# nelilepo/timetabling-ga-mpi-openmp

Hardware: AMD Instinct MI355X
Metric: fitness evals/sec (hcv+scv), pop 64K, 400-event instance; 1/2/4/8 GPUs (higher is better)
Workload: dtype i32; 1 GPU; med instance E=400 R=10 F=5 S=200 (seeded synthetic, medium01-size), population 65536 per GPU, one tt_eval (hcv+scv+feasible+penalty) per step; pop_per_gpu=65536, global_pop=65536, kernel=eval_tile5_w8, parallelism=dp1 (independent population shards)

## Files before the change

### timetabling-ga-mpi-openmp_amd/csrc/tt_common.h

```cpp
#pragma once
#include <hip/hip_runtime.h>
#include <stdint.h>

namespace ttga {

constexpr int kSlots = 45;
constexpr int kSlotsPerDay = 9;
constexpr int kMaxRooms = 64;
constexpr int kMaxSlotEvents = 256;

constexpr uint64_t kLastSlotMask = (1ull << 8) | (1ull << 17) | (1ull << 26) | (1ull << 35) | (1ull << 44);
constexpr uint64_t kTripleMask = 0x7Full | (0x7Full << 9) | (0x7Full << 18) | (0x7Full << 27) | (0x7Full << 36);

struct DevProblem {
    int E, R, S, EW;
    const int32_t* sn;
    const int32_t* stu_off;
    const int32_t* stu_ev;
    const int32_t* ev_off;
    const int32_t* ev_stu;
    const uint64_t* poss;
    const uint32_t* corr;
    int EW64;
    const uint64_t* cupT;
    const uint64_t* corr64;
    const int32_t* stc_off;
    const int32_t* stc_ev;
    const uint32_t* sid;
    const int4* srun;
    const int32_t* srun_part;
    int32_t* status;
};
constexpr int kSrunPart4 = 0, kSrunPart8 = 5, kSrunPart16 = 14, kSrunPartLen = 32;
__host__ __device__ constexpr int srun_part_base(int nw) { return nw == 4 ? kSrunPart4 : nw == 8 ? kSrunPart8 : kSrunPart16; }

__device__ __forceinline__ double pm_next(int64_t& s) {
    const int64_t IA = 16807, IM = 2147483647, IQ = 127773, IR = 2836;
    const double AM = 1.0 / 2147483647.0;
    if ((uint64_t)s <= 0x7FFFFFFFull) {
        const uint32_t u = (uint32_t)s;
        const uint32_t k32 = u / 127773u;
        int32_t t = 16807 * (int32_t)(u - k32 * 127773u) - 2836 * (int32_t)k32;
        if (t < 0) t += 2147483647;
        s = t;
        return __dmul_rn(AM, (double)t);
    }
    int64_t k = s / IQ;
    s = IA * (s - k * IQ) - IR * k;
    if (s < 0) s += IM;
    return __dmul_rn(AM, (double)s);
}

constexpr uint32_t kPmM = 2147483647u;
__device__ __forceinline__ uint32_t pm_mulmod(uint32_t a, uint32_t b) {
    const uint64_t p = (uint64_t)a * b;
    const uint32_t r = (uint32_t)(p & kPmM) + (uint32_t)(p >> 31);
    return r >= kPmM ? r - kPmM : r;
}
__device__ __forceinline__ uint32_t pm_pow(int n) {
    uint32_t r = 1, b = 16807u;
    for (; n; n >>= 1) {
        if (n & 1) r = pm_mulmod(r, b);
        b = pm_mulmod(b, b);
    }
    return r;
}

__device__ __forceinline__ int pm_pick(int64_t& s, int n) { return (int)__dmul_rn(pm_next(s), (double)n); }

__device__ __forceinline__ int mask_scv(uint64_t m) {
    int sc = __popcll(m & (m >> 1) & (m >> 2) & kTripleMask);
#pragma unroll
    for (int d = 0; d < 5; ++d) sc += (__popc((uint32_t)(m >> (9 * d)) & 0x1FFu) == 1);
    return sc;
}

__device__ __forceinline__ int wave_sum(int v) {
    v += __builtin_amdgcn_update_dpp(0, v, 0x111, 0xf, 0xf, true);
    v += __builtin_amdgcn_update_dpp(0, v, 0x112, 0xf, 0xf, true);
    v += __builtin_amdgcn_update_dpp(0, v, 0x114, 0xf, 0xf, true);
    v += __builtin_amdgcn_update_dpp(0, v, 0x118, 0xf, 0xf, true);
    v += __builtin_amdgcn_update_dpp(0, v, 0x142, 0xa, 0xf, false);
    v += __builtin_amdgcn_update_dpp(0, v, 0x143, 0xc, 0xf, false);
    return __builtin_amdgcn_readlane(v, 63);
}

__device__ __forceinline__ uint64_t ballot(bool p) { return __builtin_amdgcn_ballot_w64(p); }
__device__ __forceinline__ bool wave_any(bool p) { return __builtin_amdgcn_ballot_w64(p) != 0ull; }

__device__ __forceinline__ int wave_id() { return __builtin_amdgcn_readfirstlane((int)(threadIdx.x >> 6)); }

}
```

### timetabling-ga-mpi-openmp_amd/csrc/tt_derive.hip

```cpp
#include <hip/hip_runtime.h>

#include "tt_internal.h"

namespace ttga {
namespace {

typedef int v4i __attribute__((ext_vector_type(4)));
typedef int v16i __attribute__((ext_vector_type(16)));

__device__ __forceinline__ v4i bits_to_bytes(uint32_t h16) {
    v4i v;
#pragma unroll
    for (int d = 0; d < 4; d++) v[d] = (int)((__builtin_amdgcn_ubfe(h16, 4 * d, 4) * 0x00204081u) & 0x01010101u);
    return v;
}

struct DeriveOut {
    uint32_t* corr;
    uint32_t* corr64;
    uint32_t* cupT;
    int32_t* sn;
    uint64_t* poss;
};

// ... 44 lines not shown
    uint32_t myrow = 0u;
    uint32_t colbits = 0u;
#pragma unroll
    for (int g = 0; g < 16; g++) {
        const bool nz = acc[g] > 0;
        const uint64_t bal = ballot(nz);
        if (lane == acc_row(g, 0)) myrow = (uint32_t)bal;
        if (lane == acc_row(g, 1)) myrow = (uint32_t)(bal >> 32);
        if (nz) colbits |= 1u << acc_row(g, h);
    }
    const uint32_t col = colbits | (uint32_t)__shfl_xor((int)colbits, 32);
    if (lane < 32) {
        put_row_word(o, E, EW, EW64, i0 + lane, j0, myrow);
        if (!(diag_block && qi == qj)) put_row_word(o, E, EW, EW64, j0 + lane, i0, col);
    }
    if (diag_block && qi == qj) {
        const int c = r;
        if (h == ((c >> 2) & 1)) {
            const int reg = (c & 3) + 4 * (c >> 3);
            int v = 0;
#pragma unroll
            for (int g = 0; g < 16; g++) if (g == reg) v = acc[g];
            const int e = i0 + c;
            if (e < E) {
                o.sn[e] = v;
                uint64_t pm = 0ull;
                for (int rr = 0; rr < R; rr++) {
                    if (room_size[rr] < v) continue;
                    bool ok = true;
                    for (int f = 0; f < FW; f++) ok &= (efw[(size_t)e * FW + f] & ~rfw[(size_t)rr * FW + f]) == 0ull;
                    if (ok) pm |= 1ull << rr;
                }
                o.poss[e] = pm;
            }
        }
    }
}

}

int derive_on_device(const tt_problem* p, const uint32_t* atb, const int32_t* room_size, const uint64_t* efw,
                     const uint64_t* rfw, int FW) {
    const int E = p->E, S = p->S, R = p->R;
    const DeriveLayout DL = derive_layout(E, S);
    const int nb = DL.Ep / 64;
    const size_t at_bytes = ((size_t)DL.Ep * DL.SW * 4 + 255) & ~(size_t)255;
    const size_t rs_bytes = 256 * ((sizeof(int32_t) * R + 255) / 256);
    const size_t ef_bytes = ((sizeof(uint64_t) * E * FW) + 255) & ~(size_t)255;
    const size_t rf_bytes = ((sizeof(uint64_t) * R * FW) + 255) & ~(size_t)255;
    const size_t total = at_bytes + rs_bytes + ef_bytes + rf_bytes + 256;
    uint8_t* tmp = nullptr;
    hipStream_t st = nullptr;
    TT_HIP(hipStreamCreateWithFlags(&st, hipStreamNonBlocking));
    hipError_t he = hipMalloc(&tmp, total);
    if (he == hipErrorOutOfMemory) {
        (void)hipGetLastError();
        (void)hipStreamDestroy(st);
        set_error("tt_problem_create: the " + std::to_string(total >> 20) +
                  " MiB derivation image (E x S attendance bits) does not fit in device memory");
        return TT_ERR_LIMIT;
    }
    if (he != hipSuccess) { (void)hipStreamDestroy(st); return check_hip(he, "derive: hipMalloc"); }
    uint32_t* dAt = (uint32_t*)tmp;
    int32_t* drs = (int32_t*)(tmp + at_bytes);
    uint64_t* def = (uint64_t*)((uint8_t*)drs + rs_bytes);
    uint64_t* drf = (uint64_t*)((uint8_t*)def + ef_bytes);
    const DevProblem& d = p->dev;
    DeriveOut o{const_cast<uint32_t*>(d.corr), (uint32_t*)const_cast<uint64_t*>(d.corr64),
                (uint32_t*)const_cast<uint64_t*>(d.cupT), const_cast<int32_t*>(d.sn), const_cast<uint64_t*>(d.poss)};
    if (DL.SW > 0) he = hipMemcpyAsync(dAt, atb, (size_t)DL.Ep * DL.SW * 4, hipMemcpyHostToDevice, st);
    if (he == hipSuccess) he = hipMemcpyAsync(drs, room_size, sizeof(int32_t) * R, hipMemcpyHostToDevice, st);
    if (he == hipSuccess && FW > 0) he = hipMemcpyAsync(def, efw, sizeof(uint64_t) * E * FW, hipMemcpyHostToDevice, st);
    if (he == hipSuccess && FW > 0) he = hipMemcpyAsync(drf, rfw, sizeof(uint64_t) * R * FW, hipMemcpyHostToDevice, st);
    if (he == hipSuccess)
        hipLaunchKernelGGL(derive_corr_kernel, dim3(nb * (nb + 1) / 2), dim3(256), 0, st, dAt, E, DL.Sp, nb, drs, R, def,
                           drf, FW, o);
    if (he == hipSuccess) he = hipGetLastError();
    if (he == hipSuccess) he = hipStreamSynchronize(st);
    (void)hipFree(tmp);
    (void)hipStreamDestroy(st);
    return check_hip(he, "derive_on_device");
}

}
```

### timetabling-ga-mpi-openmp_amd/csrc/tt_eval.hip

```cpp
#include <algorithm>
#include <type_traits>
#include <utility>
#include <vector>

#include "tt_internal.h"

namespace ttga {

typedef __attribute__((address_space(4))) const uint32_t ConstU32;
typedef __attribute__((address_space(4))) const int32_t ConstI32;
typedef __attribute__((address_space(3))) unsigned long long LdsU64;


__device__ __forceinline__ int bcnt_acc(uint32_t x, int acc) {
    int r;
    asm("v_bcnt_u32_b32 %0, %1, %2" : "=v"(r) : "v"(x), "v"(acc));
    return r;
}
__device__ __forceinline__ int popc_acc(uint64_t x, int acc) {
    int r, t;
    asm("v_bcnt_u32_b32 %0, %1, %2" : "=v"(t) : "v"((uint32_t)x), "v"(acc));
    asm("v_bcnt_u32_b32 %0, %1, %2" : "=v"(r) : "v"((uint32_t)(x >> 32)), "v"(t));
    return r;
}
// ... 154 lines not shown
        }
    }
    if constexpr (K == 2) {
        if (cnt & 1) {
            uint32_t r[N / 2];
            sload_rec<N / 2>(q + steps * ST, r);
            sc += students_scv<N, 1, GAP>(my, r);
        }
    }
    return sc;
}
__device__ __noinline__ int run_scv_any(const uint8_t* my, const ConstU32* p, int cnt, int n, bool gap) {
    int sc = 0;
    for (int i = 0; i < cnt; ++i) {
        uint64_t m = 0;
        for (int j = 0; j < n / 2; ++j) {
            const uint32_t d = p[i * (n / 2) + j];
            m |= 1ull << (my[d & 0xFFFFu] & 63);
            m |= 1ull << (my[d >> 16] & 63);
        }
        sc += gap ? mask_scv_gap(m) : mask_scv(m);
    }
    return sc;
}
template <int KMAX, bool GAP = false>
__device__ __forceinline__ int lane_scv_runs(const uint8_t* my, const DevProblem& pb, int r0, int r1) {
    const ConstI32* runs = (const ConstI32*)pb.srun;
    int sc = 0;
    for (int k = r0; k < r1; ++k) {
        const int n = runs[4 * k], off = runs[4 * k + 1], cnt = runs[4 * k + 2];
        const uint32_t* p = pb.sid + off;
        switch (n) {
#define TT_RUN(N) case N: sc += run_scv<N, KMAX, GAP>(my, p, cnt); break;
            TT_RUN(2) TT_RUN(4) TT_RUN(6) TT_RUN(8) TT_RUN(10) TT_RUN(12) TT_RUN(14) TT_RUN(16)
            TT_RUN(18) TT_RUN(20) TT_RUN(22) TT_RUN(24) TT_RUN(26) TT_RUN(28) TT_RUN(30) TT_RUN(32)
#undef TT_RUN
            default: sc += run_scv_any(my, (const ConstU32*)p, cnt, n, GAP); break;
        }
    }
    return sc;
}

#ifndef TT_EVAL_ABLATE
#define TT_EVAL_ABLATE 0
#endif
__host__ __device__ inline int t5_cnt_bytes(int R) {
    return kSlots * ((R + 1) / 2) * 4;
}

struct Tile5Layout {
    int SP, WS;
    size_t tile_bytes, off_ws, off_part, bytes;
};

__host__ __device__ inline Tile5Layout tile5_layout(int E, int R, int NW, bool DB = false) {
    Tile5Layout L;
    int sp = (E + 1 + 3) & ~3;
    if (((sp >> 2) & 1) == 0) sp += 4;
    L.SP = sp;
    const int ew64 = (E + 63) / 64;
    const int cntb = t5_cnt_bytes(R);
    L.WS = (kSlots * ew64 * 8 + cntb + 15) & ~15;
    L.tile_bytes = ((size_t)64 * sp + 15) & ~(size_t)15;
    L.off_ws = (DB ? 2 : 1) * L.tile_bytes;
    L.off_part = L.off_ws + (size_t)NW * L.WS;
    L.bytes = L.off_part + 4 * (size_t)(NW * 64 + 64);
    return L;
}

template <int NW>
__device__ __forceinline__ void tile_dma(const uint8_t* src, uint8_t* dst, int np, int E, int SP, int wv, int lane) {
    const int qd = E >> 2;
    const __amdgpu_buffer_rsrc_t rs = __builtin_amdgcn_make_buffer_rsrc((void*)src, 0, np * E, 0x00020000);
    for (int r = wv; r < np; r += NW) {
        if (lane < qd)
            __builtin_amdgcn_raw_ptr_buffer_load_lds(rs, (__attribute__((address_space(3))) void*)(dst + r * SP), 4,
                                                     4 * lane, r * E, 0, 0);
        if (lane + 64 < qd)
            __builtin_amdgcn_raw_ptr_buffer_load_lds(rs, (__attribute__((address_space(3))) void*)(dst + r * SP + 256),
                                                     4, 4 * lane + 256, r * E, 0, 0);
    }
}

#ifdef TT_T5_STAMP
constexpr int kT5Launches = 8, kT5MaxBlocks = 16384, kT5Words = 10;
__device__ unsigned long long g_t5_stamp[kT5Launches * kT5MaxBlocks * kT5Words];
#endif

__device__ __forceinline__ uint32_t mad_u16_hi(uint32_t a, uint32_t b, uint32_t c) {
    uint32_t d;
    asm("v_mad_u32_u16 %0, %1, %2, %3 op_sel:[0,1,0,0]" : "=v"(d) : "v"(a), "v"(b), "v"(c));
    return d;
}

constexpr uint32_t kT5ClrBias = 0x8000u;
constexpr size_t kT5ClrReach = 0x10000u + kT5ClrBias;
constexpr int t5_clear_max(int EWC, int PK) {
    return (kSlots * EWC * 8 + kSlots * (PK == 1 ? 8 : PK == 2 ? 16 : 32) * 4 + 15) / 256;
}
template <int MAXF>
__device__ __forceinline__ void t5_clear_pieces(uint32_t m0v, uint32_t skip) {
    uint32_t keep;
    asm volatile("s_mov_b32 %[keep], m0\n"
                 "s_mov_b32 m0, %[base]\n"
                 "s_getpc_b64 vcc\n"
                 "s_add_u32 vcc_lo, vcc_lo, %[skip]\n"
                 "s_addc_u32 vcc_hi, vcc_hi, 0\n"
                 "s_setpc_b64 vcc\n"
                 ".set tt_clr_k, %c[n]\n"
                 ".rept %c[n]\n"
                 ".set tt_clr_k, tt_clr_k-1\n"
                 "ds_write_addtid_b32 %[z] offset:tt_clr_k*256\n"
                 ".endr\n"
                 "s_branch .Ltt_clr_end%=\n"
                 ".set tt_clr_k, %c[n]\n"
                 ".rept %c[n]\n"
                 ".set tt_clr_k, tt_clr_k-1\n"
                 "ds_write_addtid_b32 %[z] offset:tt_clr_k*256+%c[bias]\n"
                 ".endr\n"
                 ".Ltt_clr_end%=:\n"
                 "s_mov_b32 m0, %[keep]\n"
                 "s_nop 0"
                 : [keep] "=&s"(keep)
                 : [base] "s"(m0v), [skip] "s"(skip), [z] "v"(0u), [n] "i"(MAXF), [bias] "i"(kT5ClrBias)
                 : "memory", "scc", "vcc");
}

constexpr int kT5PrioLane = 3;
constexpr uint32_t kT5PrioW = 0x00112233u;
template <int EWC, int NW, int PK, bool DB = false>
__global__ __launch_bounds__(64 * NW, 4) void eval_tile5_kernel(DevProblem pb, const uint8_t* __restrict__ slot,
                                                              const uint8_t* __restrict__ room, int P,
                                                              int32_t* __restrict__ hcv_out,
                                                              int32_t* __restrict__ scv_out,
                                                              uint8_t* __restrict__ feas_out,
                                                              int32_t* __restrict__ pen_out, int ablate_arg) {
    extern __shared__ __attribute__((aligned(16))) uint8_t lds[];
    const int ablate = TT_EVAL_ABLATE ? ablate_arg : (ablate_arg & 3);
    constexpr int NT = 64 * NW;
#ifdef TT_T5_STAMP
    unsigned long long* st_rec =
        g_t5_stamp + ((size_t)((ablate_arg >> 8) & (kT5Launches - 1)) * kT5MaxBlocks + (blockIdx.x % kT5MaxBlocks)) * kT5Words;
    if (threadIdx.x == 0) {
        const unsigned long long t0 = __builtin_amdgcn_s_memrealtime();
        unsigned hw, xcc;
        asm volatile("s_getreg_b32 %0, hwreg(HW_REG_HW_ID)" : "=s"(hw));
        asm volatile("s_getreg_b32 %0, hwreg(HW_REG_XCC_ID)" : "=s"(xcc));
        st_rec[0] = t0;
        st_rec[1] = ((unsigned long long)xcc << 32) | hw;
    }
#endif
    const int E = pb.E, R = pb.R;
    const int lane = threadIdx.x & 63, wv = wave_id();
    const Tile5Layout L = tile5_layout(E, R, NW, DB);
    const int SP = L.SP;
    uint8_t* tile = lds;
    uint8_t* ws = lds + L.off_ws + (size_t)wv * L.WS;
    uint64_t* B = (uint64_t*)ws;
    uint32_t* cnt = (uint32_t*)(B + kSlots * EWC);
    int32_t* part = (int32_t*)(lds + L.off_part);
    int32_t* hq = part + NW * 64;
    const int tiles = (P + 63) / 64;
    const bool last_partial = E < 64 * EWC;
    const int RW = (R + 1) / 2;
    constexpr int CLRF = t5_clear_max(EWC, PK);
    const uint32_t ws_a = (uint32_t)__builtin_amdgcn_readfirstlane((int)lds_addr(ws));
    const bool ws_hi = ws_a >= 0x10000u;
    const uint32_t clr_m0 = ws_hi ? ws_a - kT5ClrBias : ws_a;
    const uint32_t clr_skip = 12u + 8u * (uint32_t)(CLRF - min(L.WS >> 8, CLRF)) + (ws_hi ? 8u * CLRF + 4u : 0u);

    using PossT = typename std::conditional<PK == 0, uint64_t, uint32_t>::type;
    uint64_t inv_cup[EWC][EWC];
    PossT inv_poss[EWC];
    uint32_t inv_ps[EWC];
    int inv_sn[EWC];
#pragma unroll
    for (int r = 0; r < EWC; ++r) {
        const int e = lane + 64 * r;
        const bool ok = e < E;
        if constexpr (PK == 1) {
            inv_ps[r] = ok ? ((~(uint32_t)pb.poss[e] & 0xFFFFu) | ((uint32_t)pb.sn[e] << 16)) : 0u;
        } else {
            inv_poss[r] = ok ? (PossT)pb.poss[e] : (PossT)~0ull;
            inv_sn[r] = ok ? pb.sn[e] : 0;
        }
#pragma unroll
        for (int w = 0; w < EWC; ++w) inv_cup[r][w] = (w >= r && ok) ? pb.cupT[(size_t)w * E + e] : 0ull;
    }
    const ConstI32* ptab = (const ConstI32*)pb.srun_part;
    const int pbase = srun_part_base(NW);
    const int r0 = ptab[pbase + wv], r1 = ptab[pbase + wv + 1];
    const bool wide = (E & 15) == 0 && (((uintptr_t)slot) & 15) == 0;
    const int qpr = E >> 4;
    const uint32_t qinv = ((1u << 20) + (uint32_t)qpr - 1) / (uint32_t)max(qpr, 1);

    if constexpr (DB) {
        if (threadIdx.x < 128) lds[(threadIdx.x >> 6) * L.tile_bytes + (threadIdx.x & 63) * SP + E] = 63;
        if (blockIdx.x < tiles)
            tile_dma<NW>(slot + (long)blockIdx.x * 64 * E, lds, (int)min(64L, (long)P - (long)blockIdx.x * 64), E, SP,
                         wv, lane);
    }
    int it = 0;
    for (int tl = blockIdx.x; tl < tiles; tl += gridDim.x, ++it) {
        const long p0 = (long)tl * 64;
        const int np = (int)min((long)64, (long)P - p0);
        const uint8_t* src = slot + p0 * E;
        if constexpr (DB) {
            tile = lds + (it & 1) * L.tile_bytes;
            asm volatile("s_waitcnt vmcnt(0)" ::: "memory");
            __syncthreads();
            const int tn = tl + gridDim.x;
            if (tn < tiles)
                tile_dma<NW>(slot + (long)tn * 64 * E, lds + ((it + 1) & 1) * L.tile_bytes,
                             (int)min(64L, (long)P - (long)tn * 64), E, SP, wv, lane);
        } else {
        __syncthreads();
        if (wide) {
            const uint4* s16 = (const uint4*)src;
#pragma unroll 2
            for (int w = threadIdx.x; w < np * qpr; w += NT) {
                const int r = (int)(((uint32_t)w * qinv) >> 20), c = w - r * qpr;
                const uint4 v = s16[w];
                uint32_t* d = (uint32_t*)(tile + r * SP + 16 * c);
                d[0] = v.x; d[1] = v.y; d[2] = v.z; d[3] = v.w;
            }
        } else {
#pragma unroll 1
            for (int r = wv; r < np; r += NW)
#pragma unroll 1
                for (int c = lane; c < E; c += 64) tile[r * SP + c] = src[(long)r * E + c];
        }
        if (threadIdx.x < 64) tile[threadIdx.x * SP + E] = 63;
        __syncthreads();
        }

        uint32_t lsp;
        asm volatile("v_mul_u32_u24 %0, %1, %2" : "=v"(lsp) : "v"(lane), "s"(SP));
        __builtin_amdgcn_s_setprio(kT5PrioLane);
        const int sc = (!(ablate & 1) && r0 < r1) ? lane_scv_runs<1>(tile + lsp, pb, r0, r1) : 0;
        part[wv * 64 + lane] = sc;

        const int nq = (ablate & 2) ? 0 : np;
        uint32_t pfn[EWC];
        const __amdgpu_buffer_rsrc_t rrs =
            __builtin_amdgcn_make_buffer_rsrc((void*)(room + p0 * E), 0, 64 * E, 0x00020000);
        auto load_row = [&](int q, uint32_t* dst) {
#pragma unroll
            for (int r = 0; r < EWC; ++r)
                dst[r] = (!last_partial || r < EWC - 1 || lane + 64 * r < E)
                             ? (uint32_t)__builtin_amdgcn_raw_buffer_load_b8(rrs, lane + 64 * r, q * E, 0)
                             : 0u;
        };
        if (wv < nq) load_row(wv, pfn);
        for (int q = wv; q < nq; q += NW) {
            const uint32_t pr = (kT5PrioW >> (4 * min((q - wv) / NW, 7))) & 3u;
            if (pr == 0) __builtin_amdgcn_s_setprio(0);
            else if (pr == 1) __builtin_amdgcn_s_setprio(1);
            else if (pr == 2) __builtin_amdgcn_s_setprio(2);
            else __builtin_amdgcn_s_setprio(3);
            uint32_t rv[EWC], sv[EWC];
#pragma unroll
            for (int r = 0; r < EWC; ++r) rv[r] = pfn[r];
            const uint8_t* rs = tile + q * SP;
#pragma unroll
            for (int r = 0; r < EWC; ++r)
                sv[r] = (!last_partial || r < EWC - 1 || lane + 64 * r < E) ? rs[lane + 64 * r] : 0u;
            if (q + NW < nq) load_row(q + NW, pfn);
            uint32_t smax = 0, rmax = 0;
#pragma unroll
            for (int r = 0; r < EWC; ++r) { smax = max(smax, sv[r]); rmax = max(rmax, rv[r]); }
            const bool any_bad = wave_any(smax >= (uint32_t)kSlots || rmax >= (uint32_t)R);
            int h = 0, last = 0;
            if (!any_bad) {
                uint32_t row[EWC];
#pragma unroll
                for (int r = 0; r < EWC; ++r) row[r] = lds_addr(B) + __umul24(sv[r], (uint32_t)(EWC * 8));
                if (!(ablate & 32)) {
                    t5_clear_pieces<CLRF>(clr_m0, clr_skip);
                    *(uint32_t*)(ws + L.WS - 256 + 4 * lane) = 0u;
                }
                __builtin_amdgcn_fence(__ATOMIC_RELEASE, "wavefront");
                __builtin_amdgcn_wave_barrier();
                __builtin_amdgcn_fence(__ATOMIC_ACQUIRE, "wavefront");
#pragma unroll
                for (int r = 0; r < EWC; ++r) {
                    if (r < EWC - 1 || !last_partial || lane + 64 * r < E) {
                        const uint32_t s = sv[r], ro = rv[r];
                        if (!(ablate & 8))
                            __hip_atomic_fetch_or((LdsU64*)(uintptr_t)row[r] + r, 1ull << lane, __ATOMIC_RELAXED,
                                                  __HIP_MEMORY_SCOPE_AGENT);
                        if (!(ablate & 16)) {
                            uint32_t* c = (uint32_t*)((uint8_t*)cnt + ((__umul24(s, (uint32_t)(2 * RW)) + (ro & ~1u)) << 1));
                            const uint32_t sh = ro << 4;
                            h += (int)__builtin_amdgcn_ubfe(atomicAdd(c, 1u << (sh & 31u)), sh, 16);
                        }
                        const bool last_slot = (kLastSlotMask >> s) & 1ull;
                        if constexpr (PK == 1) {
                            h += (int)__builtin_amdgcn_ubfe(inv_ps[r], ro, 1);
                            last = (int)mad_u16_hi((uint32_t)(kLastSlotMask >> s) & 1u, inv_ps[r], (uint32_t)last);
                        } else {
                            h += (int)(((inv_poss[r] >> ro) & 1u) ^ 1u);
                            last += last_slot ? inv_sn[r] : 0;
                        }
                    }
                }
                __builtin_amdgcn_fence(__ATOMIC_RELEASE, "wavefront");
                __builtin_amdgcn_wave_barrier();
                __builtin_amdgcn_fence(__ATOMIC_ACQUIRE, "wavefront");
                if (!(ablate & 4)) {
                    corr_words<0, EWC>(row, inv_cup, h);
                }
                if (!wave_any(h >= 1024 || last >= 1024)) {
                    const uint32_t t = (uint32_t)wave_sum((h << 16) | last);
                    h = (int)(t >> 16);
                    last = (int)(t & 0xFFFFu);
                } else {
// ... 423 lines not shown
static int auto_variant(const tt_problem* p) {
    if (tile5_fits(p, 8)) return 8;
    if (tile5_fits(p, 4)) return 7;
    if (wide_fits(p)) return 13;
    return 2;
}

extern "C" int tt_eval_auto_variant(const tt_problem* p) { return p ? auto_variant(p) : -1; }

#ifdef TT_T5_STAMP
extern "C" int tt_t5_stamp_read(unsigned long long* out, int reset) {
    TT_HIP(hipDeviceSynchronize());
    TT_HIP(hipMemcpyFromSymbol(out, HIP_SYMBOL(g_t5_stamp), sizeof(g_t5_stamp)));
    if (reset) {
        std::vector<unsigned long long> z(sizeof(g_t5_stamp) / 8, 0ull);
        TT_HIP(hipMemcpyToSymbol(HIP_SYMBOL(g_t5_stamp), z.data(), sizeof(g_t5_stamp)));
    }
    return kT5Launches * kT5MaxBlocks;
}
#endif

extern "C" int tt_eval_variant(const tt_problem* p, const uint8_t* slot, const uint8_t* room, int P, int32_t* hcv,
                               int32_t* scv, uint8_t* feasible, int32_t* penalty, int variant, void* stream) {
    int rc = check_pop_args(p, P, slot, room);
    if (rc) return rc;
    if (P > 0 && (!hcv || !scv || !feasible || !penalty)) { set_error("null output buffer"); return TT_ERR_INVALID; }
    const int ablate = variant >> 4;
    variant &= 15;
    if (variant != 0 && variant != 2 && variant != 7 && variant != 8 && variant != 13) {
        set_error("unknown eval variant (0 auto, 2 block, 7/8 tile5, 13 wide)");
        return TT_ERR_INVALID;
    }
    if (P == 0) return TT_OK;
    rc = use_device(p);
    if (rc) return rc;
    hipStream_t st = (hipStream_t)stream;
    const int E = p->E, R = p->R;
    if (variant == 0) variant = auto_variant(p);
    if (variant == 13) {
        if (!wide_fits(p)) { set_error("instance outside the wide eval path"); return TT_ERR_LIMIT; }
        const int EW64 = p->dev.EW64;
        const int tiles = (P + 63) / 64;
        {
            const size_t lds_l = lanes_lds_bytes(E);
            auto launch_l = [&](auto kern) -> int {
                int per_cu = 0;
                TT_HIP(hipOccupancyMaxActiveBlocksPerMultiprocessor(&per_cu, kern, 1024, lds_l));
                per_cu = std::min(per_cu, lds_resident_limit(lds_l));
                const int grid = std::min(tiles, std::max(1, per_cu) * p->num_cus);
                hipLaunchKernelGGL(kern, dim3(grid), dim3(1024), lds_l, st, p->dev, slot, P, scv);
                return TT_OK;
            };
            rc = launch_l(eval_lanes_kernel<16>);
            if (rc) return rc;
        }
        if (ablate & 4) return check_hip(hipGetLastError(), "tt_eval launch");
        const int NB = corr_nb(E, R, EW64);
        const CorrLayout CL = corr_layout(E, R, EW64, NB);
        auto launch = [&](auto kern) -> int {
            int per_cu = 0;
            TT_HIP(hipOccupancyMaxActiveBlocksPerMultiprocessor(&per_cu, kern, 64 * CL.NWV, CL.bytes));
            per_cu = std::min(per_cu, lds_resident_limit(CL.bytes));
            const long batches = ((long)P + NB - 1) / NB;
            const int grid = (int)std::min<long>(batches, (long)std::max(1, per_cu) * p->num_cus);
            hipLaunchKernelGGL(kern, dim3(grid), dim3(64 * CL.NWV), CL.bytes, st, p->dev, slot, room, P, hcv, scv,
                               feasible, penalty, ablate);
            return TT_OK;
        };
        if (CL.EPL <= 2)
            rc = NB == 8 ? launch(eval_corr_kernel<8, 2>) : NB == 4 ? launch(eval_corr_kernel<4, 2>) : launch(eval_corr_kernel<2, 2>);
        else
            rc = NB == 8 ? launch(eval_corr_kernel<8, kCorrMaxEPL>)
                 : NB == 4 ? launch(eval_corr_kernel<4, kCorrMaxEPL>) : launch(eval_corr_kernel<2, kCorrMaxEPL>);
        if (rc) return rc;
    } else if (variant == 7 || variant == 8) {
        const int NW = variant == 7 ? 4 : 8;
        const Tile5Layout L0 = tile5_layout(E, R, NW, false), L1 = tile5_layout(E, R, NW, true);
        const bool db_ok = (E & 3) == 0 && (((uintptr_t)slot) & 3) == 0 && L1.bytes <= 160 * 1024 &&
                           L1.off_part <= kT5ClrReach;
        if (p->dev.EW64 > 7 || L0.bytes > 160 * 1024 || L0.off_part > kT5ClrReach || E > 32767) {
            set_error("instance too large for the tile5 kernel");
            return TT_ERR_LIMIT;
        }
        const int max_sn = p->max_sn;
        const int pk = (R <= 16 && max_sn <= 0xFFFF) ? 1 : R <= 32 ? 2 : 0;
        const int tiles = (P + 63) / 64;
        auto occupancy = [&](auto kern, size_t bytes, bool two) -> int {
            std::atomic<int>& c = const_cast<tt_problem*>(p)->t5_occ[NW == 8][two];
            int per_cu = c.load(std::memory_order_relaxed);
            if (per_cu >= 0) return per_cu;
            if (hipOccupancyMaxActiveBlocksPerMultiprocessor(&per_cu, kern, 64 * NW, bytes) != hipSuccess) {
                (void)hipGetLastError();
                return 0;
            }
            per_cu = std::min(per_cu, lds_resident_limit(bytes));
            c.store(per_cu, std::memory_order_relaxed);
            return per_cu;
        };
        auto launch = [&](auto kern, size_t bytes, bool two) -> int {
            const int per_cu = occupancy(kern, bytes, two);
            const bool persist = (ablate & 64) || (two && !(ablate & 128));
            const int grid = persist ? std::min(tiles, std::max(1, per_cu) * p->num_cus) : tiles;
            hipLaunchKernelGGL(kern, dim3(grid), dim3(64 * NW), bytes, st, p->dev, slot, room, P, hcv, scv,
                               feasible, penalty, ablate);
            return TT_OK;
        };
#define TT_T5U(EWC, NWV, PKV)                                                                                      \
    {                                                                                                              \
        const bool db = db_ok && occupancy(eval_tile5_kernel<EWC, NWV, PKV, true>, L1.bytes, true) >=              \
                                     occupancy(eval_tile5_kernel<EWC, NWV, PKV, false>, L0.bytes, false);          \
        rc = db ? launch(eval_tile5_kernel<EWC, NWV, PKV, true>, L1.bytes, true)                                   \
                : launch(eval_tile5_kernel<EWC, NWV, PKV, false>, L0.bytes, false);                                \
    }
#define TT_T5N(EWC, NWV) \
    if (pk == 1) { TT_T5U(EWC, NWV, 1) } else if (pk == 2) { TT_T5U(EWC, NWV, 2) } else { TT_T5U(EWC, NWV, 0) }
#define TT_T5(EWC)                                                      \
    case EWC:                                                           \
        if (NW == 4) { TT_T5N(EWC, 4) } else { TT_T5N(EWC, 8) }         \
        break;
        switch (p->dev.EW64) {
            TT_T5(1) TT_T5(2) TT_T5(3) TT_T5(4) TT_T5(5) TT_T5(6) TT_T5(7)
            default: rc = TT_ERR_LIMIT; break;
        }
#undef TT_T5
#undef TT_T5N
#undef TT_T5U
        if (rc) return rc;
    } else {
        const size_t lds = block_lds_bytes(E, R);
        if (lds > 160 * 1024) { set_error("instance too large for the block kernel"); return TT_ERR_LIMIT; }
        hipLaunchKernelGGL(eval_block_kernel, dim3(P), dim3(kBlockThreads), lds, st, p->dev, slot, room, P, hcv,
                           scv, feasible, penalty);
    }
    return check_hip(hipGetLastError(), "tt_eval launch");
}

extern "C" int tt_eval(const tt_problem* p, const uint8_t* slot, const uint8_t* room, int P, int32_t* hcv,
                       int32_t* scv, uint8_t* feasible, int32_t* penalty, void* stream) {
    return tt_eval_variant(p, slot, room, P, hcv, scv, feasible, penalty, 0, stream);
}
```

### timetabling-ga-mpi-openmp_amd/csrc/tt_internal.h

```cpp
#pragma once
#include <hip/hip_runtime.h>
#include <stdint.h>
#include <atomic>
#include <mutex>
#include <string>
#include <vector>

#include "../../include/ttga.h"
#include "tt_common.h"

struct tt_problem {
    int E, R, F, S, device, num_cus;
    std::vector<int32_t> student_number;
    std::vector<uint64_t> poss_bits;
    std::vector<uint32_t> corr_bits;
    int nnz_students;
    void* dev_block;
    ttga::DevProblem dev;
    struct LsRedo {
        void* stream;
        int32_t* list;
        int cap;
        unsigned long long* ph_dev = nullptr;
        volatile unsigned long long* ph_host = nullptr;
        hipEvent_t ev[2] = {nullptr, nullptr};
        long calls = 0;
        int sms_last = 0;
    };
    std::vector<LsRedo> ls_redo;
    std::mutex ls_mu;
    std::atomic<int> ls_smask[2] = {-1, -1};
    std::atomic<int> t5_occ[2][2] = {{-1, -1}, {-1, -1}};
    int max_sn = 0;
};

namespace ttga {

void set_error(const std::string& msg);

int check_hip(hipError_t e, const char* what);

#define TT_HIP(call)                                         \
    do {                                                     \
        int _rc = ::ttga::check_hip((call), #call);          \
        if (_rc != TT_OK) return _rc;                        \
    } while (0)

inline int lds_resident_limit(size_t lds_bytes) {
    const size_t blocks = (lds_bytes + 1279) / 1280;
    return blocks == 0 ? 1 << 30 : (int)(128 / blocks);
}

int check_pop_args(const tt_problem* p, int P, const void* a, const void* b);

int use_device(const tt_problem* p);

struct DeriveLayout {
    int Ep, Sp, SW;
};
inline DeriveLayout derive_layout(int E, int S) {
    DeriveLayout L;
    L.Ep = (E + 63) & ~63;
    L.Sp = (S + 127) & ~127;
    L.SW = L.Sp / 32;
    return L;
}

int derive_on_device(const tt_problem* p, const uint32_t* atb, const int32_t* room_size, const uint64_t* efw,
                     const uint64_t* rfw, int FW);

}
```

### timetabling-ga-mpi-openmp_amd/csrc/tt_problem.hip

```cpp
#include <algorithm>
#include <cstring>
#include <string>
#include <vector>

#include "tt_internal.h"

namespace ttga {

static thread_local std::string g_last_error;

void set_error(const std::string& msg) { g_last_error = msg; }

int check_hip(hipError_t e, const char* what) {
    if (e == hipSuccess) return TT_OK;
    set_error(std::string(what) + ": " + hipGetErrorString(e));
    return TT_ERR_DEVICE;
}

int check_pop_args(const tt_problem* p, int P, const void* a, const void* b) {
    if (!p) { set_error("null tt_problem"); return TT_ERR_INVALID; }
    if (P < 0) { set_error("negative population size"); return TT_ERR_INVALID; }
    if (P > 0 && (!a || !b)) { set_error("null population buffer"); return TT_ERR_INVALID; }
    return TT_OK;
}
// ... 52 lines not shown

    for (int e = 0; e < E; e++) ev_off[e + 1] = ev_off[e] + degree[e];
    ev_stu.resize(stu_ev.size());
    {
        std::vector<int32_t> cur(ev_off.begin(), ev_off.end() - 1);
        for (int s = 0; s < S; s++)
            for (int k = stu_off[s]; k < stu_off[s + 1]; k++) ev_stu[cur[stu_ev[k]]++] = s;
    }
    const int FW = (F + 63) / 64;
    std::vector<uint64_t> efw((size_t)E * FW, 0ull), rfw((size_t)R * FW, 0ull);
    for (int e = 0; e < E; e++)
        for (int f = 0; f < F; f++)
            if (event_feat[(size_t)e * F + f]) efw[(size_t)e * FW + (f >> 6)] |= 1ull << (f & 63);
    for (int r = 0; r < R; r++)
        for (int f = 0; f < F; f++)
            if (room_feat[(size_t)r * F + f]) rfw[(size_t)r * FW + (f >> 6)] |= 1ull << (f & 63);
    std::vector<int32_t> stc_off(S + 1, 0), stc_ev;
    for (int s = 0; s < S; s++) {
        for (int k = stu_off[s]; k < stu_off[s + 1]; k++) stc_ev.push_back(stu_ev[k]);
        while (stc_ev.size() % 8) stc_ev.push_back(E);
        stc_off[s + 1] = (int32_t)stc_ev.size();
    }
    if (stc_ev.empty()) stc_ev.assign(8, E);
    std::vector<uint16_t> sid;
    std::vector<int32_t> srun_flat;
    std::vector<int32_t> srun_part(kSrunPartLen, 0);
    if (E <= 32767) {
        std::vector<int> order;
        for (int s = 0; s < S; s++)
            if (stu_off[s + 1] > stu_off[s]) order.push_back(s);
        auto padded = [&](int s) { const int n = stu_off[s + 1] - stu_off[s]; return n + (n & 1); };
        std::stable_sort(order.begin(), order.end(), [&](int a, int b) { return padded(a) < padded(b); });
        std::vector<int32_t> first(order.size() + 1, 0);
        std::vector<long> cost(order.size() + 1, 0);
        for (size_t i = 0; i < order.size(); i++) {
            const int s = order[i];
            first[i] = (int32_t)(sid.size() / 2);
            for (int k = stu_off[s]; k < stu_off[s + 1]; k++) sid.push_back((uint16_t)stu_ev[k]);
            if (sid.size() & 1) sid.push_back((uint16_t)E);
            cost[i + 1] = cost[i] + padded(s) + 8;
        }
        first[order.size()] = (int32_t)(sid.size() / 2);
        const size_t n_st = order.size();
        for (int nw : {4, 8, 16}) {
            const int base = srun_part_base(nw);
            size_t i = 0;
            for (int w = 0; w < nw; w++) {
                srun_part[base + w] = (int32_t)(srun_flat.size() / 4);
                const long target = cost[n_st] * (w + 1) / nw;
                const size_t i1 = w == nw - 1 ? n_st : std::max(i, (size_t)(std::lower_bound(cost.begin(), cost.end(), target) - cost.begin()));
                for (size_t j = i; j < i1;) {
                    const int ne = padded(order[j]);
                    size_t k = j;
                    while (k < i1 && padded(order[k]) == ne) k++;
                    srun_flat.insert(srun_flat.end(), {ne, first[j], (int32_t)(k - j), 0});
                    j = k;
                }
                i = i1;
            }
            srun_part[base + nw] = (int32_t)(srun_flat.size() / 4);
        }
    }
    sid.resize(sid.size() + 32, (uint16_t)E);
    if (srun_flat.empty()) srun_flat.assign(4, 0);
    p->nnz_students = (int)stu_ev.size();

    struct Part { const void* src; size_t bytes; size_t off; };
    std::vector<Part> parts = {
        {nullptr, sizeof(int32_t) * E, 0},
        {stu_off.data(), sizeof(int32_t) * (S + 1), 0},
        {stu_ev.data(), sizeof(int32_t) * stu_ev.size(), 0},
        {ev_off.data(), sizeof(int32_t) * (E + 1), 0},
        {ev_stu.data(), sizeof(int32_t) * ev_stu.size(), 0},
        {nullptr, sizeof(uint64_t) * E, 0},
        {nullptr, sizeof(uint32_t) * E * EW, 0},
        {nullptr, sizeof(int32_t) * 4, 0},
        {nullptr, sizeof(uint64_t) * EW64 * E, 0},
        {stc_off.data(), sizeof(int32_t) * stc_off.size(), 0},
        {stc_ev.data(), sizeof(int32_t) * stc_ev.size(), 0},
        {nullptr, sizeof(uint64_t) * E * EW64, 0},
        {sid.data(), sizeof(uint16_t) * sid.size(), 0},
        {srun_flat.data(), sizeof(int32_t) * srun_flat.size(), 0},
        {srun_part.data(), sizeof(int32_t) * srun_part.size(), 0},
    };
    size_t total = 0;
    for (auto& q : parts) { q.off = total; total += (q.bytes + 255) & ~(size_t)255; }
    total = std::max<size_t>(total, 256);

    int prev = 0;
    hipError_t he = hipGetDevice(&prev);
    if (he == hipSuccess) he = hipSetDevice(device);
    if (he == hipSuccess) he = hipDeviceGetAttribute(&p->num_cus, hipDeviceAttributeMultiprocessorCount, device);
    if (he == hipSuccess) he = hipMalloc(&p->dev_block, total);
    if (he != hipSuccess) { check_hip(he, "tt_problem_create"); delete p; return TT_ERR_DEVICE; }
    std::vector<uint8_t> staging(total, 0);
    for (auto& q : parts)
        if (q.src && q.bytes) memcpy(staging.data() + q.off, q.src, q.bytes);
    he = hipMemcpy(p->dev_block, staging.data(), total, hipMemcpyHostToDevice);
    if (he != hipSuccess) { check_hip(he, "tt_problem_create upload"); (void)hipFree(p->dev_block); delete p; return TT_ERR_DEVICE; }

    uint8_t* base = (uint8_t*)p->dev_block;
    DevProblem& d = p->dev;
    d.E = E; d.R = R; d.S = S; d.EW = EW;
    d.sn = (const int32_t*)(base + parts[0].off);
    d.stu_off = (const int32_t*)(base + parts[1].off);
    d.stu_ev = (const int32_t*)(base + parts[2].off);
    d.ev_off = (const int32_t*)(base + parts[3].off);
    d.ev_stu = (const int32_t*)(base + parts[4].off);
    d.poss = (const uint64_t*)(base + parts[5].off);
    d.corr = (const uint32_t*)(base + parts[6].off);
    d.status = (int32_t*)(base + parts[7].off);
    d.EW64 = EW64;
    d.cupT = (const uint64_t*)(base + parts[8].off);
    d.stc_off = (const int32_t*)(base + parts[9].off);
    d.stc_ev = (const int32_t*)(base + parts[10].off);
    d.corr64 = (const uint64_t*)(base + parts[11].off);
    d.sid = (const uint32_t*)(base + parts[12].off);
    d.srun = (const int4*)(base + parts[13].off);
    d.srun_part = (const int32_t*)(base + parts[14].off);

    int rc = TT_OK;
    he = hipSetDevice(device);
    if (he != hipSuccess) rc = check_hip(he, "tt_problem_create");
    if (rc == TT_OK) rc = derive_on_device(p, atb.data(), room_size, efw.data(), rfw.data(), FW);
    p->student_number.assign(E, 0);
    p->poss_bits.assign(E, 0ull);
    p->corr_bits.assign((size_t)E * EW, 0u);
    if (rc == TT_OK) rc = check_hip(hipMemcpy(p->student_number.data(), d.sn, sizeof(int32_t) * E, hipMemcpyDeviceToHost), "tt_problem_create readback");
    if (rc == TT_OK) rc = check_hip(hipMemcpy(p->poss_bits.data(), d.poss, sizeof(uint64_t) * E, hipMemcpyDeviceToHost), "tt_problem_create readback");
    if (rc == TT_OK) rc = check_hip(hipMemcpy(p->corr_bits.data(), d.corr, sizeof(uint32_t) * E * EW, hipMemcpyDeviceToHost), "tt_problem_create readback");
    if (rc == TT_OK && !p->student_number.empty())
        p->max_sn = *std::max_element(p->student_number.begin(), p->student_number.end());
    if (rc == TT_OK && p->student_number != degree) {
        set_error("tt_problem_create: device studentNumber differs from the attendance counts");
        rc = TT_ERR_DEVICE;
    }
    (void)hipSetDevice(prev);
    if (rc != TT_OK) {
        (void)hipFree(p->dev_block);
        delete p;
        return rc;
    }
    *out = p;
    return TT_OK;
}

int tt_problem_destroy(tt_problem* p) {
    if (!p) return TT_OK;
    int rc = TT_OK;
    if (p->dev_block) {
        int prev = 0;
        (void)hipGetDevice(&prev);
        (void)hipSetDevice(p->device);
        if (!p->ls_redo.empty()) {
            (void)hipDeviceSynchronize();
            for (auto& r : p->ls_redo) {
                (void)hipFreeAsync(r.list, nullptr);
                if (r.ph_dev) (void)hipFreeAsync(r.ph_dev, nullptr);
            }
            (void)hipDeviceSynchronize();
            for (auto& r : p->ls_redo) {
                if (r.ph_host) (void)hipHostFree((void*)r.ph_host);
                for (hipEvent_t e : r.ev)
                    if (e) (void)hipEventDestroy(e);
            }
        }
        rc = check_hip(hipFree(p->dev_block), "tt_problem_destroy");
        (void)hipSetDevice(prev);
    }
    delete p;
    return rc;
}

int tt_problem_dims(const tt_problem* p, int32_t* dims) {
    if (!p || !dims) { set_error("null argument"); return TT_ERR_INVALID; }
    dims[0] = p->E; dims[1] = p->R; dims[2] = p->F; dims[3] = p->S;
    return TT_OK;
}

int tt_problem_derived(const tt_problem* p, int32_t* student_number, int32_t* corr, int32_t* possible) {
    if (!p) { set_error("null tt_problem"); return TT_ERR_INVALID; }
    const int E = p->E, R = p->R, EW = (E + 31) / 32;
    if (student_number) std::copy(p->student_number.begin(), p->student_number.end(), student_number);
    if (corr)
        for (int i = 0; i < E; i++)
            for (int j = 0; j < E; j++) corr[(size_t)i * E + j] = (p->corr_bits[(size_t)i * EW + (j >> 5)] >> (j & 31)) & 1u;
    if (possible)
        for (int i = 0; i < E; i++)
            for (int j = 0; j < R; j++) possible[(size_t)i * R + j] = (int32_t)((p->poss_bits[i] >> j) & 1ull);
    return TT_OK;
}

int tt_device_status(const tt_problem* p, int32_t* status) {
    if (!p || !status) { set_error("null argument"); return TT_ERR_INVALID; }
    int rc = use_device(p);
    if (rc) return rc;
    TT_HIP(hipDeviceSynchronize());
    TT_HIP(hipMemcpy(status, p->dev.status, sizeof(int32_t), hipMemcpyDeviceToHost));
    return TT_OK;
}

}
```

Measured before the change: 978.5 million evals/s.

## Precompute packed per-block invariant image and DMA it into LDS at kernel start

At problem creation a device kernel packs the upper-triangular conflict words (cupT), room-possibility bits and student counts into one contiguous, lane-ordered image. The tile5 eval kernel now loads its per-lane invariants from this image, either by buffer-load-to-LDS DMA into the second tile buffer before the first tile is consumed, or directly from global memory. This replaces scattered strided gathers from cupT, poss and sn at every block start. It also restructures the first-tile staging and sync for both the double-buffered and single-buffered paths, which adds an extra DMA and barriers per block and costs some extra device memory.

```diff
diff --git a/timetabling-ga-mpi-openmp_amd/csrc/tt_common.h b/timetabling-ga-mpi-openmp_amd/csrc/tt_common.h
--- a/timetabling-ga-mpi-openmp_amd/csrc/tt_common.h
+++ b/timetabling-ga-mpi-openmp_amd/csrc/tt_common.h
@@ -30,7 +30,13 @@
     const int4* srun;
     const int32_t* srun_part;
     int32_t* status;
+    const uint8_t* t5_img;
+    int t5_img_bytes;
 };
+__host__ __device__ constexpr int t5_img_corr_rows(int EWC) { return EWC * (EWC + 1) / 2; }
+__host__ __device__ constexpr int t5_img_bytes(int EWC, int PK) {
+    return 512 * t5_img_corr_rows(EWC) + EWC * (PK == 1 ? 256 : PK == 2 ? 512 : 768);
+}
 constexpr int kSrunPart4 = 0, kSrunPart8 = 5, kSrunPart16 = 14, kSrunPartLen = 32;
 __host__ __device__ constexpr int srun_part_base(int nw) { return nw == 4 ? kSrunPart4 : nw == 8 ? kSrunPart8 : kSrunPart16; }
 
diff --git a/timetabling-ga-mpi-openmp_amd/csrc/tt_derive.hip b/timetabling-ga-mpi-openmp_amd/csrc/tt_derive.hip
--- a/timetabling-ga-mpi-openmp_amd/csrc/tt_derive.hip
+++ b/timetabling-ga-mpi-openmp_amd/csrc/tt_derive.hip
@@ -150,4 +150,38 @@
     return check_hip(he, "derive_on_device");
 }
 
+namespace {
+
+__global__ __launch_bounds__(64) void t5_image_kernel(DevProblem d, int pk, uint8_t* img) {
+    const int E = d.E, EWC = d.EW64, r = blockIdx.x, lane = threadIdx.x;
+    const int e = 64 * r + lane;
+    const bool ok = e < E;
+    uint64_t* c = (uint64_t*)img + (size_t)(r * EWC - r * (r - 1) / 2) * 64 + lane;
+    for (int w = r; w < EWC; ++w) c[(w - r) * 64] = ok ? d.cupT[(size_t)w * E + e] : 0ull;
+    uint8_t* ev = img + 512 * t5_img_corr_rows(EWC);
+    const uint64_t poss = ok ? d.poss[e] : ~0ull;
+    const int32_t sn = ok ? d.sn[e] : 0;
+    if (pk == 1) {
+        ((uint32_t*)ev)[e] = ok ? ((~(uint32_t)poss & 0xFFFFu) | ((uint32_t)sn << 16)) : 0u;
+    } else if (pk == 2) {
+        ((uint32_t*)ev)[e] = (uint32_t)poss;
+        ((int32_t*)(ev + 256 * EWC))[e] = sn;
+    } else {
+        ((uint64_t*)ev)[e] = poss;
+        ((int32_t*)(ev + 512 * EWC))[e] = sn;
+    }
 }
+
+}
+
+int build_t5_image(tt_problem* p) {
+    DevProblem& d = p->dev;
+    if (!d.t5_img) return TT_OK;
+    const int pk = t5_pk(p->R, p->max_sn);
+    d.t5_img_bytes = t5_img_bytes(d.EW64, pk);
+    hipLaunchKernelGGL(t5_image_kernel, dim3(d.EW64), dim3(64), 0, nullptr, d, pk, const_cast<uint8_t*>(d.t5_img));
+    TT_HIP(hipGetLastError());
+    return check_hip(hipStreamSynchronize(nullptr), "build_t5_image");
+}
+
+}
diff --git a/timetabling-ga-mpi-openmp_amd/csrc/tt_eval.hip b/timetabling-ga-mpi-openmp_amd/csrc/tt_eval.hip
--- a/timetabling-ga-mpi-openmp_amd/csrc/tt_eval.hip
+++ b/timetabling-ga-mpi-openmp_amd/csrc/tt_eval.hip
@@ -260,6 +260,32 @@
     }
 }
 
+template <int NW>
+__device__ __forceinline__ void image_dma(const uint8_t* img, int bytes, uint8_t* dst, int wv, int lane) {
+    const __amdgpu_buffer_rsrc_t rs = __builtin_amdgcn_make_buffer_rsrc((void*)img, 0, bytes, 0x00020000);
+    for (int k = wv; k < (bytes >> 8); k += NW)
+        __builtin_amdgcn_raw_ptr_buffer_load_lds(rs, (__attribute__((address_space(3))) void*)(dst + 256 * k), 4,
+                                                 4 * lane, 256 * k, 0, 0);
+}
+
+template <int EWC, int PK, typename PossT>
+__device__ __forceinline__ void t5_load_inv(const uint8_t* img, int lane, uint64_t (*cup)[EWC], uint32_t* ps,
+                                            PossT* poss, int* sn) {
+    const uint64_t* c = (const uint64_t*)img + lane;
+    const uint8_t* ev = img + 512 * t5_img_corr_rows(EWC);
+#pragma unroll
+    for (int r = 0; r < EWC; ++r) {
+#pragma unroll
+        for (int w = 0; w < EWC; ++w) cup[r][w] = w >= r ? c[64 * (r * EWC - r * (r - 1) / 2 + w - r)] : 0ull;
+        if constexpr (PK == 1) {
+            ps[r] = ((const uint32_t*)ev)[64 * r + lane];
+        } else {
+            poss[r] = ((const PossT*)ev)[64 * r + lane];
+            sn[r] = ((const int*)(ev + EWC * 64 * sizeof(PossT)))[64 * r + lane];
+        }
+    }
+}
+
 #ifdef TT_T5_STAMP
 constexpr int kT5Launches = 8, kT5MaxBlocks = 16384, kT5Words = 10;
 __device__ unsigned long long g_t5_stamp[kT5Launches * kT5MaxBlocks * kT5Words];
@@ -352,19 +378,8 @@
     PossT inv_poss[EWC];
     uint32_t inv_ps[EWC];
     int inv_sn[EWC];
-#pragma unroll
-    for (int r = 0; r < EWC; ++r) {
-        const int e = lane + 64 * r;
-        const bool ok = e < E;
-        if constexpr (PK == 1) {
-            inv_ps[r] = ok ? ((~(uint32_t)pb.poss[e] & 0xFFFFu) | ((uint32_t)pb.sn[e] << 16)) : 0u;
-        } else {
-            inv_poss[r] = ok ? (PossT)pb.poss[e] : (PossT)~0ull;
-            inv_sn[r] = ok ? pb.sn[e] : 0;
-        }
-#pragma unroll
-        for (int w = 0; w < EWC; ++w) inv_cup[r][w] = (w >= r && ok) ? pb.cupT[(size_t)w * E + e] : 0ull;
-    }
+    auto load_inv = [&](const uint8_t* img) { t5_load_inv<EWC, PK, PossT>(img, lane, inv_cup, inv_ps, inv_poss, inv_sn); };
+    const bool img_lds = DB && (size_t)pb.t5_img_bytes <= L.tile_bytes;
     const ConstI32* ptab = (const ConstI32*)pb.srun_part;
     const int pbase = srun_part_base(NW);
     const int r0 = ptab[pbase + wv], r1 = ptab[pbase + wv + 1];
@@ -373,26 +388,22 @@
     const uint32_t qinv = ((1u << 20) + (uint32_t)qpr - 1) / (uint32_t)max(qpr, 1);
 
     if constexpr (DB) {
-        if (threadIdx.x < 128) lds[(threadIdx.x >> 6) * L.tile_bytes + (threadIdx.x & 63) * SP + E] = 63;
+        if (threadIdx.x < 64) lds[threadIdx.x * SP + E] = 63;
         if (blockIdx.x < tiles)
             tile_dma<NW>(slot + (long)blockIdx.x * 64 * E, lds, (int)min(64L, (long)P - (long)blockIdx.x * 64), E, SP,
                          wv, lane);
-    }
-    int it = 0;
-    for (int tl = blockIdx.x; tl < tiles; tl += gridDim.x, ++it) {
-        const long p0 = (long)tl * 64;
-        const int np = (int)min((long)64, (long)P - p0);
-        const uint8_t* src = slot + p0 * E;
-        if constexpr (DB) {
-            tile = lds + (it & 1) * L.tile_bytes;
+        if (img_lds) {
+            image_dma<NW>(pb.t5_img, pb.t5_img_bytes, lds + L.tile_bytes, wv, lane);
             asm volatile("s_waitcnt vmcnt(0)" ::: "memory");
             __syncthreads();
-            const int tn = tl + gridDim.x;
-            if (tn < tiles)
-                tile_dma<NW>(slot + (long)tn * 64 * E, lds + ((it + 1) & 1) * L.tile_bytes,
-                             (int)min(64L, (long)P - (long)tn * 64), E, SP, wv, lane);
+            load_inv(lds + L.tile_bytes);
+            __syncthreads();
         } else {
-        __syncthreads();
+            load_inv(pb.t5_img);
+        }
+        if (threadIdx.x < 64) lds[L.tile_bytes + threadIdx.x * SP + E] = 63;
+    }
+    auto stage = [&](const uint8_t* src, int np) {
         if (wide) {
             const uint4* s16 = (const uint4*)src;
 #pragma unroll 2
@@ -409,7 +420,33 @@
                 for (int c = lane; c < E; c += 64) tile[r * SP + c] = src[(long)r * E + c];
         }
         if (threadIdx.x < 64) tile[threadIdx.x * SP + E] = 63;
-        __syncthreads();
+    };
+    if constexpr (!DB) {
+        if (blockIdx.x < tiles)
+            stage(slot + (long)blockIdx.x * 64 * E, (int)min(64L, (long)P - (long)blockIdx.x * 64));
+        load_inv(pb.t5_img);
+    }
+    int it = 0;
+    for (int tl = blockIdx.x; tl < tiles; tl += gridDim.x, ++it) {
+        const long p0 = (long)tl * 64;
+        const int np = (int)min((long)64, (long)P - p0);
+        const uint8_t* src = slot + p0 * E;
+        if constexpr (DB) {
+            tile = lds + (it & 1) * L.tile_bytes;
+            if (!(img_lds && it == 0)) {
+                asm volatile("s_waitcnt vmcnt(0)" ::: "memory");
+                __syncthreads();
+            }
+            const int tn = tl + gridDim.x;
+            if (tn < tiles)
+                tile_dma<NW>(slot + (long)tn * 64 * E, lds + ((it + 1) & 1) * L.tile_bytes,
+                             (int)min(64L, (long)P - (long)tn * 64), E, SP, wv, lane);
+        } else {
+            if (it > 0) {
+                __syncthreads();
+                stage(src, np);
+            }
+            __syncthreads();
         }
 
         uint32_t lsp;
@@ -999,8 +1036,7 @@
             set_error("instance too large for the tile5 kernel");
             return TT_ERR_LIMIT;
         }
-        const int max_sn = p->max_sn;
-        const int pk = (R <= 16 && max_sn <= 0xFFFF) ? 1 : R <= 32 ? 2 : 0;
+        const int pk = t5_pk(R, p->max_sn);
         const int tiles = (P + 63) / 64;
         auto occupancy = [&](auto kern, size_t bytes, bool two) -> int {
             std::atomic<int>& c = const_cast<tt_problem*>(p)->t5_occ[NW == 8][two];
diff --git a/timetabling-ga-mpi-openmp_amd/csrc/tt_internal.h b/timetabling-ga-mpi-openmp_amd/csrc/tt_internal.h
--- a/timetabling-ga-mpi-openmp_amd/csrc/tt_internal.h
+++ b/timetabling-ga-mpi-openmp_amd/csrc/tt_internal.h
@@ -69,4 +69,8 @@
 int derive_on_device(const tt_problem* p, const uint32_t* atb, const int32_t* room_size, const uint64_t* efw,
                      const uint64_t* rfw, int FW);
 
+inline int t5_pk(int R, int max_sn) { return (R <= 16 && max_sn <= 0xFFFF) ? 1 : R <= 32 ? 2 : 0; }
+
+int build_t5_image(tt_problem* p);
+
 }
diff --git a/timetabling-ga-mpi-openmp_amd/csrc/tt_problem.hip b/timetabling-ga-mpi-openmp_amd/csrc/tt_problem.hip
--- a/timetabling-ga-mpi-openmp_amd/csrc/tt_problem.hip
+++ b/timetabling-ga-mpi-openmp_amd/csrc/tt_problem.hip
@@ -158,6 +158,7 @@
         {sid.data(), sizeof(uint16_t) * sid.size(), 0},
         {srun_flat.data(), sizeof(int32_t) * srun_flat.size(), 0},
         {srun_part.data(), sizeof(int32_t) * srun_part.size(), 0},
+        {nullptr, EW64 <= 7 ? (size_t)t5_img_bytes(EW64, 0) : 0, 0},
     };
     size_t total = 0;
     for (auto& q : parts) { q.off = total; total += (q.bytes + 255) & ~(size_t)255; }
@@ -194,6 +195,8 @@
     d.sid = (const uint32_t*)(base + parts[12].off);
     d.srun = (const int4*)(base + parts[13].off);
     d.srun_part = (const int32_t*)(base + parts[14].off);
+    d.t5_img = parts[15].bytes ? base + parts[15].off : nullptr;
+    d.t5_img_bytes = 0;
 
     int rc = TT_OK;
     he = hipSetDevice(device);
@@ -211,6 +214,7 @@
         set_error("tt_problem_create: device studentNumber differs from the attendance counts");
         rc = TT_ERR_DEVICE;
     }
+    if (rc == TT_OK) rc = build_t5_image(p);
     (void)hipSetDevice(prev);
     if (rc != TT_OK) {
         (void)hipFree(p->dev_block);
```

Measured after the change: 1.013 billion evals/s (median of 6 runs). +3.5%, better.
